# ZhangT-tech/MoCA-Video

Hardware: AMD Instinct MI355X
Metric: denoising UNet-steps/sec @16x320x512 fp16 (higher is better)
Workload: dtype f16

## Files before the change

### include/moca_hip.h

```cpp
#ifndef MOCA_HIP_H
#define MOCA_HIP_H

#include <stdint.h>

#ifdef __cplusplus
extern "C" {
#endif

#define MOCA_OK            0
#define MOCA_E_BADARG     -1
#define MOCA_E_LAUNCH     -2
#define MOCA_E_NODEVICE   -3
#define MOCA_E_GRAPH      -4

#define MOCA_A_LINEAR   0
#define MOCA_A_CONV3X3  1
#define MOCA_A_TCONV3   2

#define MOCA_EP_GEGLU   1
#define MOCA_EP_OUT_F32 2
#define MOCA_FORCE_SMALL_TILE 4
#define MOCA_EP_COLSUM 16
#define MOCA_EP_LN     32
#define MOCA_EP_GELU    8
// ... 227 lines not shown
int moca_base_ddim_step_f32(moca_fifo_state* state, float* x, const float* eps_c, const float* eps_u, const float* noise,
                            float* pred_x0, const float* coef, int32_t S, float cfg_scale, int32_t use_scale, int64_t n, void* stream);
int moca_mask_frame_sums_f32(const float* mask, float* sums, int32_t frames, int32_t HW, void* stream);

int moca_freq_mix_3d_f32(const float* x, const float* noise, const float* lpf, float* out,
                         int32_t C, int32_t T, int32_t H, int32_t W, float* ws, void* stream);
int64_t moca_freq_mix_ws_bytes(int32_t C, int32_t T, int32_t H, int32_t W);
int moca_freq_filter_f32(float* lpf, int32_t T, int32_t H, int32_t W, int32_t type, int32_t n,
                         double d_s, double d_t, void* stream);

int moca_graph_begin(void* stream);
int moca_graph_end(void* stream, void** graph_exec_out);
int moca_graph_launch(void* graph_exec, void* stream);
int moca_graph_destroy(void* graph_exec);
int moca_stream_create(void** stream_out);
int moca_stream_destroy(void* stream);
int moca_stream_sync(void* stream);
int moca_event_create(void** ev_out);
int moca_event_record(void* ev, void* stream);
int moca_event_elapsed_ms(void* ev_start, void* ev_stop, float* ms_out);
int moca_event_destroy(void* ev);

#define MOCA_TUNE_GEMM_W80   0
#define MOCA_TUNE_GEMM_G4    1
#define MOCA_TUNE_GEMM_SQ256 2
#define MOCA_TUNE_GEMM_WIDE  3
#define MOCA_TUNE_GN_SLAB    4
#define MOCA_TUNE_GEMM_G4P   5
#define MOCA_TUNE_GEMM_MF32  6
#define MOCA_TUNE_GEMM_SQP   7
#define MOCA_TUNE_SQP_WALK   8
#define MOCA_TUNE_SLAB_F16   9
#define MOCA_TUNE_GEMM_WS    10
#define MOCA_TUNE_COUNT      11
int moca_set_tuning(int32_t knob, int32_t value);
int moca_debug_clock_sampler(void* buf, int32_t blocks, int32_t nsamples, const int32_t* stop, void* stream);

int moca_device_info(char* name, int32_t len, int32_t* cu_count);
const char* moca_version(void);

#ifdef __cplusplus
}
#endif
#endif
```

### moca_video_amd/csrc/norm.hip

```cpp
#include "common.h"

namespace {

constexpr int GN_GROUPS = 32;

__host__ __device__ inline int gn_nchunk(int F, int HW) {
    int n = 2048 / (F > 0 ? F : 1);
    if (n < 1) n = 1;
    const int maxc = (HW + 7) / 8;
    if (n > maxc) n = maxc;
    if (n < 1) n = 1;
    return n;
}

__global__ void gn_partial_kernel(const half_t* __restrict__ x, float* __restrict__ partial,
                                  int HW, int C, int nchunk) {
    extern __shared__ __attribute__((aligned(16))) char smem_raw[];
    float* s_sum = reinterpret_cast<float*>(smem_raw);
    float* s_sq = s_sum + blockDim.y * C;
    const int f = blockIdx.x, chunk = blockIdx.y;
    const int cx = threadIdx.x, py = threadIdx.y, ppb = blockDim.y;
    const int pc = (HW + nchunk - 1) / nchunk;
    const int p_begin = chunk * pc, p_end = min(p_begin + pc, HW);
    float s[8], q[8];
#pragma unroll
    for (int j = 0; j < 8; ++j) { s[j] = 0.f; q[j] = 0.f; }
    const half_t* base = x + ((int64_t)f * HW) * C + cx * 8;
    int pp = p_begin + py;
    for (; pp + 3 * ppb < p_end; pp += 4 * ppb) {
        half8v v[4];
#pragma unroll
        for (int u = 0; u < 4; ++u) v[u] = *reinterpret_cast<const half8v*>(base + (int64_t)(pp + u * ppb) * C);
#pragma unroll
        for (int u = 0; u < 4; ++u)
#pragma unroll
            for (int j = 0; j < 8; ++j) { const float a = (float)v[u][j]; s[j] += a; q[j] += a * a; }
    }
    for (; pp < p_end; pp += ppb) {
        const half8v v = *reinterpret_cast<const half8v*>(base + (int64_t)pp * C);
#pragma unroll
        for (int j = 0; j < 8; ++j) { const float a = (float)v[j]; s[j] += a; q[j] += a * a; }
    }
#pragma unroll
    for (int j = 0; j < 8; ++j) { s_sum[py * C + cx * 8 + j] = s[j]; s_sq[py * C + cx * 8 + j] = q[j]; }
    __syncthreads();
    const int tid = py * blockDim.x + cx;
// ... 37 lines not shown
        float2 v[4];
#pragma unroll
        for (int u = 0; u < 4; ++u) {
            const int i = i0 + u * FIN_T;
            v[u] = i < n ? *reinterpret_cast<const float2*>(base + ((int64_t)i * GN_GROUPS + g) * 2) : float2{0.f, 0.f};
        }
#pragma unroll
        for (int u = 0; u < 4; ++u) { a += (double)v[u].x; b += (double)v[u].y; }
    }
    gn_finalize_store(a, b, meanrstd, (int64_t)sg * GN_GROUPS + g, inv_count, eps);
}

__global__ __launch_bounds__(FIN_T) void gn_finalize_colsum_kernel(const float* __restrict__ colsum, float* __restrict__ meanrstd,
                                                                   int tps, int C, int cpg, double inv_count, float eps) {
    const int sg = blockIdx.x, g = blockIdx.y, l = threadIdx.x;
    const int n = tps * cpg;
    double a = 0.0, b = 0.0;
    for (int i0 = l; i0 < n; i0 += 4 * FIN_T) {
        float2 v[4];
#pragma unroll
        for (int u = 0; u < 4; ++u) {
            const int i = i0 + u * FIN_T;
            const int t = i / cpg, c = g * cpg + (i - t * cpg);
            v[u] = i < n ? *reinterpret_cast<const float2*>(colsum + (((int64_t)sg * tps + t) * C + c) * 2) : float2{0.f, 0.f};
        }
#pragma unroll
        for (int u = 0; u < 4; ++u) { a += (double)v[u].x; b += (double)v[u].y; }
    }
    gn_finalize_store(a, b, meanrstd, (int64_t)sg * GN_GROUPS + g, inv_count, eps);
}

__global__ void gn_apply_kernel(const half_t* __restrict__ x, half_t* __restrict__ y,
                                const float* __restrict__ gamma, const float* __restrict__ beta,
                                const float* __restrict__ meanrstd, int HW, int C, int nchunk,
                                int frames_per_stat, int silu) {
    const int f = blockIdx.x, chunk = blockIdx.y;
    const int cx = threadIdx.x, py = threadIdx.y, ppb = blockDim.y;
    const int pc = (HW + nchunk - 1) / nchunk;
    const int p_begin = chunk * pc, p_end = min(p_begin + pc, HW);
    if (p_begin >= p_end) return;
    const int cpg = C / GN_GROUPS;
    const int sg = f / frames_per_stat;
    const int64_t off = ((int64_t)f * HW) * C + cx * 8;
    auto load4 = [&](half8v (&v)[4], int pp) {
#pragma unroll
        for (int u = 0; u < 4; ++u) v[u] = *reinterpret_cast<const half8v*>(x + off + (int64_t)min(pp + u * ppb, p_end - 1) * C);
    };
    int pp = p_begin + py;
    half8v cur[4], nxt[4];
    load4(cur, pp);
    float sc[8], sh[8];
#pragma unroll
    for (int j = 0; j < 8; ++j) {
        const int c = cx * 8 + j;
        const int g = c / cpg;
        const float mean = meanrstd[((int64_t)sg * GN_GROUPS + g) * 2];
        const float rstd = meanrstd[((int64_t)sg * GN_GROUPS + g) * 2 + 1];
        sc[j] = rstd * gamma[c];
        sh[j] = beta[c] - mean * sc[j];
    }
    auto norm8 = [&](const half8v& v) {
        half8v o;
#pragma unroll
        for (int j = 0; j < 8; ++j) {
            float a = (float)v[j] * sc[j] + sh[j];
            if (silu) a = moca_silu(a);
            o[j] = (half_t)a;
        }
        return o;
    };
    for (; pp < p_end; pp += 4 * ppb) {
        const bool more = pp + 4 * ppb < p_end;
        if (more) load4(nxt, pp + 4 * ppb);
#pragma unroll
        for (int u = 0; u < 4; ++u)
            if (pp + u * ppb < p_end) *reinterpret_cast<half8v*>(y + off + (int64_t)(pp + u * ppb) * C) = norm8(cur[u]);
        if (more) {
#pragma unroll
            for (int u = 0; u < 4; ++u) cur[u] = nxt[u];
        }
    }
}

template <bool STREAM>
__device__ __forceinline__ void gn_st8(half_t* ptr, const half8v v) {
    if constexpr (STREAM) __builtin_nontemporal_store(v, reinterpret_cast<half8v*>(ptr));
    else *reinterpret_cast<half8v*>(ptr) = v;
}
template <bool STREAM>
__global__ void gn_apply_gstat_kernel(const half_t* __restrict__ x, half_t* __restrict__ y,
                                      const float* __restrict__ gamma, const float* __restrict__ beta,
                                      const int64_t* __restrict__ gstat, int HW, int C, int nchunk,
                                      int frames_per_stat, double inv_count, float eps, int silu) {
    __shared__ float s_mr[2 * GN_GROUPS];
    const int f = blockIdx.x, chunk = blockIdx.y;
    const int cx = threadIdx.x, py = threadIdx.y, ppb = blockDim.y;
    const int tid = py * blockDim.x + cx;
    const int pc = (HW + nchunk - 1) / nchunk;
    const int p_begin = chunk * pc, p_end = min(p_begin + pc, HW);
    if (p_begin >= p_end) return;
    const int cpg = C / GN_GROUPS;
    const int sg = f / frames_per_stat;
    const int64_t off = ((int64_t)f * HW) * C + cx * 8;
    auto load4 = [&](half8v (&v)[4], int pp) {
#pragma unroll
        for (int u = 0; u < 4; ++u) v[u] = *reinterpret_cast<const half8v*>(x + off + (int64_t)min(pp + u * ppb, p_end - 1) * C);
    };
    int pp = p_begin + py;
    half8v cur[4], nxt[4];
    load4(cur, pp);
    const f32x4 gm0 = *reinterpret_cast<const f32x4*>(gamma + cx * 8), gm1 = *reinterpret_cast<const f32x4*>(gamma + cx * 8 + 4);
    const f32x4 bt0 = *reinterpret_cast<const f32x4*>(beta + cx * 8), bt1 = *reinterpret_cast<const f32x4*>(beta + cx * 8 + 4);
    if (tid < GN_GROUPS) {
        const double a = moca_gstat_get(gstat + ((int64_t)sg * GN_GROUPS + tid) * 2, 0), b = moca_gstat_get(gstat + ((int64_t)sg * GN_GROUPS + tid) * 2 + 1, 1);
        const double mean = a * inv_count;
        double var = b * inv_count - mean * mean;
        if (var < 0.0) var = 0.0;
        s_mr[2 * tid] = (float)mean;
        s_mr[2 * tid + 1] = (float)(1.0 / sqrt(var + (double)eps));
    }
    __syncthreads();
    float sc[8], sh[8];
#pragma unroll
    for (int j = 0; j < 8; ++j) {
        const int c = cx * 8 + j;
        const int g = c / cpg;
        sc[j] = s_mr[2 * g + 1] * (j < 4 ? gm0[j & 3] : gm1[j & 3]);
        sh[j] = (j < 4 ? bt0[j & 3] : bt1[j & 3]) - s_mr[2 * g] * sc[j];
    }
    auto norm8 = [&](const half8v& v) {
        half8v o;
#pragma unroll
        for (int j = 0; j < 8; ++j) {
            float a = (float)v[j] * sc[j] + sh[j];
            if (silu) a = moca_silu(a);
            o[j] = (half_t)a;
// ... 38 lines not shown
        for (int u = 0; u < 4; ++u) v[u] = *reinterpret_cast<const half8v*>(src + (int64_t)(pp + u * ppb) * ld);
#pragma unroll
        for (int u = 0; u < 4; ++u) {
            gn_st8<STREAM>(dst + (int64_t)(pp + u * ppb) * C, v[u]);
#pragma unroll
            for (int j = 0; j < 8; ++j) { const float t = (float)v[u][j]; s[j] += t; q[j] += t * t; }
        }
    }
    for (; pp < p_end; pp += ppb) {
        const half8v v = *reinterpret_cast<const half8v*>(src + (int64_t)pp * ld);
        gn_st8<STREAM>(dst + (int64_t)pp * C, v);
#pragma unroll
        for (int j = 0; j < 8; ++j) { const float t = (float)v[j]; s[j] += t; q[j] += t * t; }
    }
#pragma unroll
    for (int j = 0; j < 8; ++j) { s_sum[py * C + cx * 8 + j] = s[j]; s_sq[py * C + cx * 8 + j] = q[j]; }
    __syncthreads();
    const int tid = py * blockDim.x + cx;
    if (tid < 2 * GN_GROUPS) {
        const int g = tid >> 1, comp = tid & 1;
        const int cpg = C / GN_GROUPS;
        const float* base = comp ? s_sq : s_sum;
        float t = 0.f;
        for (int y = 0; y < ppb; ++y)
            for (int c = g * cpg; c < (g + 1) * cpg; ++c) t += base[y * C + c];
        moca_gstat_add(gstat + ((int64_t)(f / frames_per_stat) * GN_GROUPS + g) * 2 + comp, comp, t);
    }
}

template <bool STREAM>
__global__ void gn_apply_gstat_cat_kernel(const half_t* __restrict__ a, const half_t* __restrict__ b, half_t* __restrict__ y,
                                          const float* __restrict__ gamma, const float* __restrict__ beta,
                                          const int64_t* __restrict__ gstat_cat, const int64_t* __restrict__ gstat_b,
                                          int HW, int C1, int C2, int nchunk, int frames_per_stat, int sgb_mod, double inv_count, float eps, int silu) {
    __shared__ float s_mr[2 * GN_GROUPS];
    const int C = C1 + C2;
    const int f = blockIdx.x, chunk = blockIdx.y;
    const int cx = threadIdx.x, py = threadIdx.y, ppb = blockDim.y;
    const int tid = py * blockDim.x + cx;
    const int pc = (HW + nchunk - 1) / nchunk;
    const int p_begin = chunk * pc, p_end = min(p_begin + pc, HW);
    if (p_begin >= p_end) return;
    const int cpg = C / GN_GROUPS;
    const int sg = f / frames_per_stat;
    const bool from_a = cx * 8 < C1;
    const half_t* src = from_a ? a + ((int64_t)f * HW) * C1 + cx * 8 : b + ((int64_t)f * HW) * C2 + (cx * 8 - C1);
    const int ld = from_a ? C1 : C2;
    const int64_t off = ((int64_t)f * HW) * C + cx * 8;
    auto load4 = [&](half8v (&v)[4], int pp) {
#pragma unroll
        for (int u = 0; u < 4; ++u) v[u] = *reinterpret_cast<const half8v*>(src + (int64_t)min(pp + u * ppb, p_end - 1) * ld);
    };
    int pp = p_begin + py;
    half8v cur[4], nxt[4];
    load4(cur, pp);
    const f32x4 gm0 = *reinterpret_cast<const f32x4*>(gamma + cx * 8), gm1 = *reinterpret_cast<const f32x4*>(gamma + cx * 8 + 4);
    const f32x4 bt0 = *reinterpret_cast<const f32x4*>(beta + cx * 8), bt1 = *reinterpret_cast<const f32x4*>(beta + cx * 8 + 4);
    if (tid < GN_GROUPS) {
        const int64_t* ga = gstat_cat + ((int64_t)sg * GN_GROUPS + tid) * 2;
        double sa = moca_gstat_get(ga, 0), sq = moca_gstat_get(ga + 1, 1);
        if (gstat_b) {
            const int cpg2 = C2 / GN_GROUPS;
            const int lo = max(tid * cpg - C1, 0), hi = min((tid + 1) * cpg - C1, C2);
            for (int j = lo / cpg2; j * cpg2 < hi; ++j) {
                const int64_t* gb = gstat_b + ((int64_t)(sg % sgb_mod) * GN_GROUPS + j) * 2;
                sa += moca_gstat_get(gb, 0); sq += moca_gstat_get(gb + 1, 1);
            }
        }
        const double mean = sa * inv_count;
        double var = sq * inv_count - mean * mean;
        if (var < 0.0) var = 0.0;
        s_mr[2 * tid] = (float)mean;
        s_mr[2 * tid + 1] = (float)(1.0 / sqrt(var + (double)eps));
    }
    __syncthreads();
    float sc[8], sh[8];
#pragma unroll
    for (int j = 0; j < 8; ++j) {
        const int c = cx * 8 + j;
        const int g = c / cpg;
        sc[j] = s_mr[2 * g + 1] * (j < 4 ? gm0[j & 3] : gm1[j & 3]);
// ... 107 lines not shown
        if (var < 0.0) var = 0.0;
        const float rstd = (float)(1.0 / sqrt(var + (double)eps));
        const float sc = rstd * gm_t;
        s_sc[tid] = sc;
        s_sh[tid] = bt_t - (float)mean * sc;
    }
    __syncthreads();
    const int rps = (R + S - 1) / S;
    const int r0 = split * rps, r1 = min(R, r0 + rps);
    half_t* ys = y + base;
    {
        int row = r0 + tid / vpr, v = tid % vpr;
#pragma unroll 2
        for (; row < r1;) {
            const int64_t o = (int64_t)row * C + v * VEC;
            const vec_t d = *reinterpret_cast<const vec_t*>(xs + o);
            vec_t r;
#pragma unroll
            for (int j = 0; j < VEC; ++j) {
                float a = (float)d[j] * s_sc[v * VEC + j] + s_sh[v * VEC + j];
                if (silu) a = moca_silu(a);
                r[j] = (half_t)a;
            }
            *reinterpret_cast<vec_t*>(ys + o) = r;
            row += dr; v += dv;
            if (v >= vpr) { v -= vpr; ++row; }
        }
    }
}

template <int CPT>
__global__ __launch_bounds__(1024) void gn_slab_reg_kernel(const half_t* __restrict__ x, half_t* __restrict__ y,
                                                            const float* __restrict__ gamma, const float* __restrict__ beta,
                                                            int R, int C, int cpg, double inv_count, float eps, int silu) {
    __shared__ float s_red[2][16];
    __shared__ float s_sc[128], s_sh[128];
    const int tid = threadIdx.x, nthr = blockDim.x;
    const int slab = blockIdx.x, sg = slab / GN_GROUPS, g = slab % GN_GROUPS;
    const int vpr = cpg / 8, nchunks = R * vpr;
    const int64_t base = (int64_t)sg * R * C + g * cpg;
    const float gm_t = tid < cpg ? gamma[g * cpg + tid] : 0.f, bt_t = tid < cpg ? beta[g * cpg + tid] : 0.f;
    half8v v[CPT];
    int off[CPT];
    float s = 0.f, q = 0.f;
#pragma unroll
    for (int i = 0; i < CPT; ++i) {
        const int idx = tid + i * nthr;
        off[i] = -1;
        if (idx < nchunks) {
            const int row = idx / vpr, c = idx - row * vpr;
            off[i] = row * C + c * 8;
            v[i] = *reinterpret_cast<const half8v*>(x + base + off[i]);
        }
    }
#pragma unroll
    for (int i = 0; i < CPT; ++i)
        if (off[i] >= 0) {
#pragma unroll
            for (int j = 0; j < 8; ++j) { const float a = (float)v[i][j]; s += a; q += a * a; }
        }
    s = wave_sum(s); q = wave_sum(q);
    if ((tid & 63) == 0) { s_red[0][tid >> 6] = s; s_red[1][tid >> 6] = q; }
    __syncthreads();
    if (tid < cpg) {
        double a = 0.0, b = 0.0;
        for (int w = 0; w < (nthr >> 6); ++w) { a += (double)s_red[0][w]; b += (double)s_red[1][w]; }
        const double mean = a * inv_count;
        double var = b * inv_count - mean * mean;
        if (var < 0.0) var = 0.0;
        const float rstd = (float)(1.0 / sqrt(var + (double)eps));
        const float sc = rstd * gm_t;
        s_sc[tid] = sc;
        s_sh[tid] = bt_t - (float)mean * sc;
    }
    __syncthreads();
#pragma unroll
    for (int i = 0; i < CPT; ++i)
        if (off[i] >= 0) {
            const int c0 = (off[i] % C);
            half8v r;
#pragma unroll
            for (int j = 0; j < 8; ++j) {
                float a = (float)v[i][j] * s_sc[c0 + j] + s_sh[c0 + j];
                if (silu) a = moca_silu(a);
                r[j] = (half_t)a;
            }
            *reinterpret_cast<half8v*>(y + base + off[i]) = r;
        }
}

template <int MAXCH, int LN_ROWS>
__global__ __launch_bounds__(256) void layernorm_kernel(const half_t* __restrict__ x, half_t* __restrict__ y,
                                                        const float* __restrict__ gamma, const float* __restrict__ beta,
                                                        int M, int C, float eps) {
    const int lane = threadIdx.x & 63, wave = threadIdx.x >> 6;
    const int row0 = (blockIdx.x * 4 + wave) * LN_ROWS;
    if (row0 >= M) return;
    const int nch = C / 8;
    half8v v[LN_ROWS][MAXCH];
#pragma unroll
    for (int r = 0; r < LN_ROWS; ++r) {
        const int row = min(row0 + r, M - 1);
        const half_t* xr = x + (int64_t)row * C;
#pragma unroll
        for (int i = 0; i < MAXCH; ++i) {
            const int ch = lane + 64 * i;
            if (ch < nch) v[r][i] = *reinterpret_cast<const half8v*>(xr + ch * 8);
        }
    }
    float mean[LN_ROWS], rstd[LN_ROWS];
#pragma unroll
// ... 27 lines not shown
        if (ch < nch) {
            const f32x4 g0 = *reinterpret_cast<const f32x4*>(gamma + ch * 8), g1 = *reinterpret_cast<const f32x4*>(gamma + ch * 8 + 4);
            const f32x4 b0 = *reinterpret_cast<const f32x4*>(beta + ch * 8), b1 = *reinterpret_cast<const f32x4*>(beta + ch * 8 + 4);
#pragma unroll
            for (int r = 0; r < LN_ROWS; ++r) {
                if (row0 + r < M) {
                    half8v o;
#pragma unroll
                    for (int j = 0; j < 4; ++j) {
                        o[j] = (half_t)(((float)v[r][i][j] - mean[r]) * rstd[r] * g0[j] + b0[j]);
                        o[4 + j] = (half_t)(((float)v[r][i][4 + j] - mean[r]) * rstd[r] * g1[j] + b1[j]);
                    }
                    *reinterpret_cast<half8v*>(y + (int64_t)(row0 + r) * C + ch * 8) = o;
                }
            }
        }
    }
}

}

extern "C" int64_t moca_groupnorm_ws_bytes(int32_t F, int32_t HW, int32_t C) {
    (void)C;
    const int nchunk = gn_nchunk(F, HW);
    return ((int64_t)F * nchunk * GN_GROUPS * 2 + (int64_t)F * GN_GROUPS * 2) * 4;
}

extern "C" int moca_groupnorm_nhwc_f16(const void* x, void* y, const float* gamma, const float* beta,
                                       int32_t F, int32_t HW, int32_t C, int32_t frames_per_stat,
                                       float eps, int32_t silu, float* ws, void* stream) {
    if (!x || !y || !gamma || !beta || !ws) return MOCA_E_BADARG;
    if (F <= 0 || HW <= 0 || C <= 0 || C % (8 * 1) || C % GN_GROUPS || frames_per_stat <= 0 || F % frames_per_stat) return MOCA_E_BADARG;
    const int nch8 = C / 8;
    if (nch8 > 1024) return MOCA_E_BADARG;
    int ppb = 256 / nch8;
    if (ppb < 1) ppb = 1;
    const int nchunk = gn_nchunk(F, HW);
    float* partial = ws;
    float* meanrstd = ws + (int64_t)F * nchunk * GN_GROUPS * 2;
    hipStream_t st = moca_stream(stream);
    const double inv_count = 1.0 / ((double)frames_per_stat * HW * (C / GN_GROUPS));
    {
        const int slab_mode = moca_tuning_get(MOCA_TUNE_GN_SLAB);
        const int cpg = C / GN_GROUPS;
        const int64_t bytes = (int64_t)F * HW * C * 2;
        const int64_t R64 = (int64_t)frames_per_stat * HW;
        if (slab_mode && cpg % 2 == 0 && cpg <= 128 && R64 < (1 << 24) &&
            (slab_mode == 2 || bytes <= (8 << 20) || (frames_per_stat == 1 && HW <= 160 && bytes <= (28 << 20)))) {
            const int R = (int)R64;
            const int n_slabs = (F / frames_per_stat) * GN_GROUPS;
            {
                const int nchunks = R * (cpg / 8);
                if (cpg % 8 == 0 && nchunks <= 4096 && nchunks >= 256) {
                    const int cpt = (nchunks + 1023) / 1024;
                    const int thr = ((nchunks + cpt - 1) / cpt + 63) / 64 * 64;
                    const half_t* xi = reinterpret_cast<const half_t*>(x);
                    half_t* yo = reinterpret_cast<half_t*>(y);
#define MOCA_SLABREG(CPT) hipLaunchKernelGGL(gn_slab_reg_kernel<CPT>, dim3(n_slabs), dim3(thr), 0, st, xi, yo, gamma, beta, R, C, cpg, inv_count, eps, silu)
                    if (cpt == 1) MOCA_SLABREG(1); else if (cpt == 2) MOCA_SLABREG(2); else if (cpt == 3) MOCA_SLABREG(3); else MOCA_SLABREG(4);
#undef MOCA_SLABREG
                    MOCA_CHECK_LAUNCH();
                    return MOCA_OK;
                }
            }
            int S = 1024 / n_slabs;
            if (S > 16) S = 16;
            if (S > R) S = R;
            if (S < 1) S = 1;
            const int xcd_map = (n_slabs % 8 == 0) ? 1 : 0;
            const dim3 g1(n_slabs * S), b1(256);
            const half_t* xi = reinterpret_cast<const half_t*>(x);
            half_t* yo = reinterpret_cast<half_t*>(y);
            if (cpg % 8 == 0)
                hipLaunchKernelGGL(gn_slab_kernel<8>, g1, b1, 0, st, xi, yo, gamma, beta, R, C, cpg, S, xcd_map, inv_count, eps, silu);
            else if (cpg % 4 == 0)
                hipLaunchKernelGGL(gn_slab_kernel<4>, g1, b1, 0, st, xi, yo, gamma, beta, R, C, cpg, S, xcd_map, inv_count, eps, silu);
            else
                hipLaunchKernelGGL(gn_slab_kernel<2>, g1, b1, 0, st, xi, yo, gamma, beta, R, C, cpg, S, xcd_map, inv_count, eps, silu);
            MOCA_CHECK_LAUNCH();
            return MOCA_OK;
        }
    }
    const dim3 grid(F, nchunk), block(nch8, ppb);
    const size_t lds = (size_t)ppb * C * 2 * sizeof(float);
    hipLaunchKernelGGL(gn_partial_kernel, grid, block, lds, st, reinterpret_cast<const half_t*>(x), partial, HW, C, nchunk);
    MOCA_CHECK_LAUNCH();
    hipLaunchKernelGGL(gn_finalize_kernel, dim3(F / frames_per_stat, GN_GROUPS), dim3(FIN_T), 0, st, partial, meanrstd,
                       frames_per_stat, nchunk, inv_count, eps);
    MOCA_CHECK_LAUNCH();
    hipLaunchKernelGGL(gn_apply_kernel, grid, block, 0, st, reinterpret_cast<const half_t*>(x), reinterpret_cast<half_t*>(y),
                       gamma, beta, meanrstd, HW, C, nchunk, frames_per_stat, silu);
    MOCA_CHECK_LAUNCH();
    return MOCA_OK;
}

extern "C" int moca_groupnorm_colsum_f16(const void* x, void* y, const float* gamma, const float* beta, const float* colsum,
                                         int32_t tile_rows, int32_t F, int32_t HW, int32_t C, int32_t frames_per_stat,
                                         float eps, int32_t silu, float* ws, void* stream) {
    if (!x || !y || !gamma || !beta || !ws || !colsum) return MOCA_E_BADARG;
    if (F <= 0 || HW <= 0 || C <= 0 || C % 8 || C % GN_GROUPS || frames_per_stat <= 0 || F % frames_per_stat) return MOCA_E_BADARG;
    if (tile_rows <= 0 || ((int64_t)frames_per_stat * HW) % tile_rows) return MOCA_E_BADARG;
    const int nch8 = C / 8;
    if (nch8 > 1024) return MOCA_E_BADARG;
    int ppb = 256 / nch8;
    if (ppb < 1) ppb = 1;
    const int nchunk = gn_nchunk(F, HW);
    float* meanrstd = ws + (int64_t)F * nchunk * GN_GROUPS * 2;
    hipStream_t st = moca_stream(stream);
    const double inv_count = 1.0 / ((double)frames_per_stat * HW * (C / GN_GROUPS));
    const int tps = (int)(((int64_t)frames_per_stat * HW) / tile_rows);
    hipLaunchKernelGGL(gn_finalize_colsum_kernel, dim3(F / frames_per_stat, GN_GROUPS), dim3(FIN_T), 0, st, colsum, meanrstd,
                       tps, C, C / GN_GROUPS, inv_count, eps);
    MOCA_CHECK_LAUNCH();
    const dim3 grid(F, nchunk), block(nch8, ppb);
    hipLaunchKernelGGL(gn_apply_kernel, grid, block, 0, st, reinterpret_cast<const half_t*>(x), reinterpret_cast<half_t*>(y),
                       gamma, beta, meanrstd, HW, C, nchunk, frames_per_stat, silu);
    MOCA_CHECK_LAUNCH();
    return MOCA_OK;
}

extern "C" int moca_groupnorm_gstat_f16(const void* x, void* y, const float* gamma, const float* beta, const int64_t* gstat,
                                        int32_t F, int32_t HW, int32_t C, int32_t frames_per_stat,
                                        float eps, int32_t silu, void* stream) {
    if (!x || !y || !gamma || !beta || !gstat) return MOCA_E_BADARG;
    if ((reinterpret_cast<uintptr_t>(gamma) | reinterpret_cast<uintptr_t>(beta)) & 15) return MOCA_E_BADARG;
    if (F <= 0 || HW <= 0 || C <= 0 || C % 8 || C % GN_GROUPS || frames_per_stat <= 0 || F % frames_per_stat) return MOCA_E_BADARG;
    const int nch8 = C / 8;
    if (nch8 > 1024) return MOCA_E_BADARG;
    int ppb = 256 / nch8;
    if (ppb < 1) ppb = 1;
    if (nch8 * ppb < GN_GROUPS) return MOCA_E_BADARG;
    const int nchunk = gn_nchunk(F, HW);
    const double inv_count = 1.0 / ((double)frames_per_stat * HW * (C / GN_GROUPS));
    const dim3 grid(F, nchunk), block(nch8, ppb);
    const bool streams = (int64_t)F * HW * C * 2 >= (128ll << 20);
    hipLaunchKernelGGL(streams ? gn_apply_gstat_kernel<true> : gn_apply_gstat_kernel<false>, grid, block, 0, moca_stream(stream),
                       reinterpret_cast<const half_t*>(x), reinterpret_cast<half_t*>(y), gamma, beta, gstat, HW, C, nchunk, frames_per_stat,
                       inv_count, eps, silu);
    MOCA_CHECK_LAUNCH();
    return MOCA_OK;
}

__global__ __launch_bounds__(256) void gn_fold_weights_kernel(const half_t* __restrict__ w, const float* __restrict__ bias,
                                                              const float* __restrict__ gamma, const float* __restrict__ beta,
                                                              const int64_t* __restrict__ gstat, half_t* __restrict__ wg, float* __restrict__ bg,
                                                              int N, int K, int ldw, double inv_count, float eps) {
    extern __shared__ float s_st[];
    const int sg = blockIdx.x, tid = threadIdx.x;
    const int cpg = K / GN_GROUPS;
    __shared__ float s_mr[2 * GN_GROUPS];
    if (tid < GN_GROUPS) {
        const double a = moca_gstat_get(gstat + ((int64_t)sg * GN_GROUPS + tid) * 2, 0), b = moca_gstat_get(gstat + ((int64_t)sg * GN_GROUPS + tid) * 2 + 1, 1);
        const double mean = a * inv_count;
        double var = b * inv_count - mean * mean;
        if (var < 0.0) var = 0.0;
        s_mr[2 * tid] = (float)mean;
        s_mr[2 * tid + 1] = (float)(1.0 / sqrt(var + (double)eps));
    }
    __syncthreads();
    for (int k = tid; k < K; k += 256) {
        const int g = k / cpg;
        s_st[k] = s_mr[2 * g + 1] * gamma[k];
        s_st[K + k] = beta[k];
    }
    __syncthreads();
    const int cpr = ldw / 8;
    float* s_dot = s_st + 2 * K;
    const int rows_pb = 16;
    const int n0 = blockIdx.y * rows_pb;
    for (int idx = tid; idx < rows_pb * cpr; idx += 256) {
// ... 42 lines not shown
    const int C = C1 + C2;
    if (C % GN_GROUPS || frames_per_stat <= 0 || F % frames_per_stat) return MOCA_E_BADARG;
    const int nch8 = C / 8;
    if (nch8 > 1024) return MOCA_E_BADARG;
    int ppb = 256 / nch8;
    if (ppb < 1) ppb = 1;
    if (nch8 * ppb < 2 * GN_GROUPS) return MOCA_E_BADARG;
    const int nchunk = gn_nchunk(F, HW);
    const size_t lds = (size_t)ppb * C * 2 * sizeof(float);
    if (lds > 64 * 1024) return MOCA_E_BADARG;
    const bool streams = (int64_t)F * HW * C * 2 >= (128ll << 20);
    hipLaunchKernelGGL(streams ? concat_gstat_kernel<true> : concat_gstat_kernel<false>, dim3(F, nchunk), dim3(nch8, ppb), lds, moca_stream(stream),
                       reinterpret_cast<const half_t*>(a), reinterpret_cast<const half_t*>(b), reinterpret_cast<half_t*>(out), gstat, HW, C1, C2,
                       nchunk, frames_per_stat);
    MOCA_CHECK_LAUNCH();
    return MOCA_OK;
}

extern "C" int moca_groupnorm_gstat_cat_f16(const void* a, const void* b, void* y, const float* gamma, const float* beta,
                                            const int64_t* gstat_cat, const int64_t* gstat_b, int32_t Fb, int32_t F, int32_t HW, int32_t C1,
                                            int32_t C2, int32_t frames_per_stat, float eps, int32_t silu, void* stream) {
    if (!a || !b || !y || !gamma || !beta || !gstat_cat) return MOCA_E_BADARG;
    if ((reinterpret_cast<uintptr_t>(gamma) | reinterpret_cast<uintptr_t>(beta)) & 15) return MOCA_E_BADARG;
    if (Fb <= 0) Fb = F;
    if (Fb > F || F % Fb || Fb % frames_per_stat) return MOCA_E_BADARG;
    if (F <= 0 || HW <= 0 || C1 <= 0 || C2 <= 0 || C1 % 8 || C2 % 8 || frames_per_stat <= 0 || F % frames_per_stat) return MOCA_E_BADARG;
    const int C = C1 + C2;
    if (C % GN_GROUPS) return MOCA_E_BADARG;
    if (gstat_b) {
        const int cpg = C / GN_GROUPS, cpg2 = C2 / GN_GROUPS;
        if (C2 % GN_GROUPS || cpg % cpg2 || (C1 % cpg) % cpg2) return MOCA_E_BADARG;
    }
    const int nch8 = C / 8;
    if (nch8 > 1024) return MOCA_E_BADARG;
    int ppb = 256 / nch8;
    if (ppb < 1) ppb = 1;
    if (nch8 * ppb < GN_GROUPS) return MOCA_E_BADARG;
    const int nchunk = gn_nchunk(F, HW);
    const double inv_count = 1.0 / ((double)frames_per_stat * HW * (C / GN_GROUPS));
    const dim3 grid(F, nchunk), block(nch8, ppb);
    const bool streams = (int64_t)F * HW * C * 2 >= (128ll << 20);
    hipLaunchKernelGGL(streams ? gn_apply_gstat_cat_kernel<true> : gn_apply_gstat_cat_kernel<false>, grid, block, 0, moca_stream(stream),
                       reinterpret_cast<const half_t*>(a), reinterpret_cast<const half_t*>(b), reinterpret_cast<half_t*>(y), gamma, beta,
                       gstat_cat, gstat_b, HW, C1, C2, nchunk, frames_per_stat, Fb / frames_per_stat, inv_count, eps, silu);
    MOCA_CHECK_LAUNCH();
    return MOCA_OK;
}

extern "C" int moca_gstat_accum_f16(const void* x, int32_t F, int32_t HW, int32_t C, int32_t frames_per_stat, int32_t cpg, int32_t coff,
                                    int64_t* gstat, void* stream) {
    if (!x || !gstat || F <= 0 || HW <= 0 || C <= 0 || C % 8 || frames_per_stat <= 0 || F % frames_per_stat) return MOCA_E_BADARG;
    if (cpg <= 0 || coff < 0 || (coff + C - 1) / cpg >= GN_GROUPS) return MOCA_E_BADARG;
    const int nch8 = C / 8;
    if (nch8 > 1024) return MOCA_E_BADARG;
    int ppb = 256 / nch8;
    if (ppb < 1) ppb = 1;
    if (nch8 * ppb < 2 * ((coff + C - 1) / cpg - coff / cpg + 1)) return MOCA_E_BADARG;
    const int nchunk = gn_nchunk(F, HW);
    const size_t lds = (size_t)ppb * C * 2 * sizeof(float);
    if (lds > 64 * 1024) return MOCA_E_BADARG;
    hipLaunchKernelGGL(gstat_accum_kernel, dim3(F, nchunk), dim3(nch8, ppb), lds, moca_stream(stream),
                       reinterpret_cast<const half_t*>(x), gstat, HW, C, nchunk, frames_per_stat, cpg, coff);
    MOCA_CHECK_LAUNCH();
    return MOCA_OK;
}

extern "C" int moca_layernorm_f16(const void* x, void* y, const float* gamma, const float* beta,
                                  int32_t M, int32_t C, float eps, void* stream) {
    if (!x || !y || !gamma || !beta || M <= 0 || C <= 0 || C % 8) return MOCA_E_BADARG;
    const int nch = C / 8;
    hipStream_t st = moca_stream(stream);
    const half_t* xi = reinterpret_cast<const half_t*>(x);
    half_t* yo = reinterpret_cast<half_t*>(y);
    const dim3 block(256);
#define MOCA_LN(MAXCH, ROWS) hipLaunchKernelGGL((layernorm_kernel<MAXCH, ROWS>), dim3((M + 4 * ROWS - 1) / (4 * ROWS)), block, 0, st, xi, yo, gamma, beta, M, C, eps)
    if (M >= 16384) {
        if (nch <= 64) MOCA_LN(1, 4);
// ... 16 lines not shown
```

### moca_video_amd/csrc/runtime.hip

```cpp
#include "common.h"
#include <string.h>
#include <stdio.h>
#include <stdlib.h>

extern "C" int moca_graph_begin(void* stream) {
    if (hipStreamBeginCapture(moca_stream(stream), hipStreamCaptureModeThreadLocal) != hipSuccess) return MOCA_E_GRAPH;
    return MOCA_OK;
}

extern "C" int moca_graph_end(void* stream, void** graph_exec_out) {
    if (!graph_exec_out) return MOCA_E_BADARG;
    hipGraph_t g = nullptr;
    if (hipStreamEndCapture(moca_stream(stream), &g) != hipSuccess || !g) return MOCA_E_GRAPH;
    hipGraphExec_t ge = nullptr;
    hipError_t e = hipGraphInstantiate(&ge, g, nullptr, nullptr, 0);
    (void)hipGraphDestroy(g);
    if (e != hipSuccess || !ge) return MOCA_E_GRAPH;
    *graph_exec_out = reinterpret_cast<void*>(ge);
    return MOCA_OK;
}

extern "C" int moca_graph_launch(void* graph_exec, void* stream) {
    if (!graph_exec) return MOCA_E_BADARG;
    if (hipGraphLaunch(reinterpret_cast<hipGraphExec_t>(graph_exec), moca_stream(stream)) != hipSuccess) return MOCA_E_GRAPH;
// ... 65 lines not shown
    const int64_t n16 = bytes / 16;
    int blocks = (int)((n16 + 255) / 256);
    if (blocks < 1) blocks = 1;
    if (blocks > 1024) blocks = 1024;
    hipLaunchKernelGGL(zero_kernel, dim3(blocks), dim3(256), 0, moca_stream(stream), reinterpret_cast<uint4*>(ptr), n16,
                       reinterpret_cast<unsigned char*>(ptr) + n16 * 16, (int)(bytes - n16 * 16));
    MOCA_CHECK_LAUNCH();
    return MOCA_OK;
}

__global__ __launch_bounds__(64) void clock_sampler_kernel(unsigned long long* __restrict__ buf, int nsamples, const volatile int* stop) {
#if defined(__HIP_DEVICE_COMPILE__)
    if (threadIdx.x) return;
    unsigned long long* b = buf + (size_t)blockIdx.x * nsamples * 2;
    for (int i = 0; i < nsamples; ++i) {
        unsigned long long t, r;
        asm volatile("s_memtime %0\n\ts_memrealtime %1\n\ts_waitcnt lgkmcnt(0)" : "=s"(t), "=s"(r)::"memory");
        b[2 * i] = t;
        b[2 * i + 1] = r;
        if (stop && *stop) break;
        __builtin_amdgcn_s_sleep(127);
        __builtin_amdgcn_s_sleep(127);
    }
#endif
}
extern "C" int moca_debug_clock_sampler(void* buf, int32_t blocks, int32_t nsamples, const int32_t* stop, void* stream) {
    if (!buf || blocks < 1 || blocks > 64 || nsamples < 1 || nsamples > (1 << 20)) return MOCA_E_BADARG;
    hipLaunchKernelGGL(clock_sampler_kernel, dim3(blocks), dim3(64), 0, moca_stream(stream), reinterpret_cast<unsigned long long*>(buf), nsamples,
                       reinterpret_cast<const volatile int*>(stop));
    MOCA_CHECK_LAUNCH();
    return MOCA_OK;
}

static int g_tuning[MOCA_TUNE_COUNT] = {1, 1, 1, 1, 1, 1, 0, 1, 0, 0, 1};
int moca_tuning_get(int knob) { return (knob >= 0 && knob < MOCA_TUNE_COUNT) ? g_tuning[knob] : 0; }
extern "C" int moca_set_tuning(int32_t knob, int32_t value) {
    if (knob < 0 || knob >= MOCA_TUNE_COUNT || value < 0 || value > 2) return MOCA_E_BADARG;
    const int old = g_tuning[knob];
    g_tuning[knob] = value;
    return old;
}
```

### moca_video_amd/lib.py

```python
from __future__ import annotations

import ctypes as C
import os

import torch

_HERE = os.path.dirname(os.path.abspath(__file__))
LIB_PATH = os.environ.get("MOCA_HIP_LIB") or os.path.join(_HERE, "libmoca_hip.so")

MOCA_A_LINEAR, MOCA_A_CONV3X3, MOCA_A_TCONV3 = 0, 1, 2
MOCA_EP_GEGLU, MOCA_EP_OUT_F32, MOCA_FORCE_SMALL_TILE, MOCA_EP_GELU, MOCA_EP_COLSUM, MOCA_EP_LN = 1, 2, 4, 8, 16, 32
MOCA_EP_ROWSUM, MOCA_EP_LNFOLD, MOCA_EP_GSTAT, MOCA_EP_TATTN, MOCA_EP_SLABS = 64, 128, 256, 512, 1024
MOCA_TUNE_GEMM_W80, MOCA_TUNE_GEMM_G4, MOCA_TUNE_GEMM_SQ256, MOCA_TUNE_GEMM_WIDE, MOCA_TUNE_GN_SLAB, MOCA_TUNE_GEMM_G4P, MOCA_TUNE_GEMM_MF32, MOCA_TUNE_GEMM_SQP, MOCA_TUNE_SQP_WALK = 0, 1, 2, 3, 4, 5, 6, 7, 8
MOCA_TUNE_SLAB_F16 = 9
MOCA_TUNE_GEMM_WS = 10
(MOCA_ROUTE_SMALL64, MOCA_ROUTE_SMALL128, MOCA_ROUTE_GLDS128, MOCA_ROUTE_GLDS160, MOCA_ROUTE_G4, MOCA_ROUTE_W80, MOCA_ROUTE_W80W,
 MOCA_ROUTE_SQ256, MOCA_ROUTE_G4P, MOCA_ROUTE_SQP, MOCA_ROUTE_TATTN, MOCA_ROUTE_WS) = range(1, 13)

_ERR = {0: "ok", -1: "bad argument (shape/alignment contract)", -2: "HIP launch/runtime error",
        -3: "no gfx950 device", -4: "graph capture/replay failed"}


class MocaHipError(RuntimeError):
    pass


class GemmParams(C.Structure):
    _fields_ = [
        ("a", C.c_void_p), ("w", C.c_void_p), ("out", C.c_void_p), ("bias", C.c_void_p),
        ("rowadd", C.c_void_p), ("residual", C.c_void_p), ("splitk_ws", C.c_void_p),
        ("M", C.c_int32), ("N", C.c_int32), ("K", C.c_int32),
        ("lda", C.c_int32), ("ldw", C.c_int32), ("ldo", C.c_int32), ("ldr", C.c_int32), ("ld_rowadd", C.c_int32),
        ("rowadd_div", C.c_int32), ("a_mode", C.c_int32), ("C", C.c_int32),
        ("inH", C.c_int32), ("inW", C.c_int32), ("outH", C.c_int32), ("outW", C.c_int32),
        ("stride", C.c_int32), ("up", C.c_int32), ("T", C.c_int32), ("HW", C.c_int32),
        ("flags", C.c_int32), ("splits", C.c_int32), ("nopad_lo", C.c_int32), ("prefetch_kib", C.c_int32),
        ("tattn_causal", C.c_int32),
        ("colsum", C.c_void_p), ("ln_gamma", C.c_void_p), ("ln_beta", C.c_void_p), ("ln_out", C.c_void_p),
        ("ld_ln", C.c_int32), ("ln_eps", C.c_float),
        ("rowsum", C.c_void_p), ("lnf_part", C.c_void_p), ("lnf_wsum", C.c_void_p),
        ("lnf_nparts", C.c_int32), ("reserved2_", C.c_int32),
        ("gstat", C.c_void_p), ("gstat_rows", C.c_int32), ("tattn_scale", C.c_float),
        ("prefetch", C.c_void_p), ("up_phase", C.c_int32), ("reserved4_", C.c_int32),
        ("a2", C.c_void_p), ("lda2", C.c_int32), ("k1", C.c_int32), ("gstat_cpg", C.c_int32), ("gstat_coff", C.c_int32),
        ("wgroup_rows", C.c_int32), ("wgroup_stride", C.c_int32),
    ]


# ... 154 lines not shown
```

Before: 60.25.

## Regrid GroupNorm apply over stat groups and split slab-register kernel across blocks

```diff
diff --git a/include/moca_hip.h b/include/moca_hip.h
--- a/include/moca_hip.h
+++ b/include/moca_hip.h
@@ -283,7 +283,8 @@
 #define MOCA_TUNE_SQP_WALK   8
 #define MOCA_TUNE_SLAB_F16   9
 #define MOCA_TUNE_GEMM_WS    10
-#define MOCA_TUNE_COUNT      11
+#define MOCA_TUNE_GN_SLAB_SPLIT 11
+#define MOCA_TUNE_COUNT      12
 int moca_set_tuning(int32_t knob, int32_t value);
 int moca_debug_clock_sampler(void* buf, int32_t blocks, int32_t nsamples, const int32_t* stop, void* stream);
 
diff --git a/moca_video_amd/csrc/norm.hip b/moca_video_amd/csrc/norm.hip
--- a/moca_video_amd/csrc/norm.hip
+++ b/moca_video_amd/csrc/norm.hip
@@ -12,6 +12,33 @@
     if (n < 1) n = 1;
     return n;
 }
+
+struct GnApplyGeom { int ppb, R, rpb, bpsg, gps; dim3 grid; };
+inline GnApplyGeom gn_apply_geom(int nch8, int F, int HW, int fps) {
+    GnApplyGeom g;
+    int a = nch8, b = 64;
+    while (b) { const int t = a % b; a = b; b = t; }
+    g.ppb = 64 / a;
+    g.ppb *= (256 + nch8 * g.ppb - 1) / (nch8 * g.ppb);
+    if (nch8 * g.ppb > 512) g.ppb = 256 / nch8 > 0 ? 256 / nch8 : 1;
+    g.R = fps * HW; g.gps = 1;
+    g.rpb = 4 * g.ppb;
+    g.bpsg = (g.R + g.rpb - 1) / g.rpb;
+    if ((int64_t)(F / fps) * g.bpsg <= 2048) {
+        g.grid = dim3((F / fps) * g.bpsg);
+        return g;
+    }
+    const int nchunk = gn_nchunk(F, HW);
+    g.ppb = 256 / nch8 > 0 ? 256 / nch8 : 1;
+    g.R = HW; g.gps = fps;
+    g.rpb = (HW + nchunk - 1) / nchunk;
+    g.bpsg = nchunk;
+    g.grid = dim3(F, nchunk);
+    return g;
+}
+#define GN_APPLY_BLOCK() \
+    const int grp = gridDim.y > 1 ? blockIdx.x : blockIdx.x / bpsg, blk = gridDim.y > 1 ? blockIdx.y : blockIdx.x - grp * bpsg; \
+    const int sg = grp / gps
 
 __global__ void gn_partial_kernel(const half_t* __restrict__ x, float* __restrict__ partial,
                                   int HW, int C, int nchunk) {
@@ -115,16 +142,13 @@
 
 __global__ void gn_apply_kernel(const half_t* __restrict__ x, half_t* __restrict__ y,
                                 const float* __restrict__ gamma, const float* __restrict__ beta,
-                                const float* __restrict__ meanrstd, int HW, int C, int nchunk,
-                                int frames_per_stat, int silu) {
-    const int f = blockIdx.x, chunk = blockIdx.y;
+                                const float* __restrict__ meanrstd, int R, int C, int rpb, int bpsg, int gps, int silu) {
+    GN_APPLY_BLOCK();
     const int cx = threadIdx.x, py = threadIdx.y, ppb = blockDim.y;
-    const int pc = (HW + nchunk - 1) / nchunk;
-    const int p_begin = chunk * pc, p_end = min(p_begin + pc, HW);
+    const int p_begin = blk * rpb, p_end = min(p_begin + rpb, R);
     if (p_begin >= p_end) return;
     const int cpg = C / GN_GROUPS;
-    const int sg = f / frames_per_stat;
-    const int64_t off = ((int64_t)f * HW) * C + cx * 8;
+    const int64_t off = ((int64_t)grp * R) * C + cx * 8;
     auto load4 = [&](half8v (&v)[4], int pp) {
 #pragma unroll
         for (int u = 0; u < 4; ++u) v[u] = *reinterpret_cast<const half8v*>(x + off + (int64_t)min(pp + u * ppb, p_end - 1) * C);
@@ -173,18 +197,16 @@
 template <bool STREAM>
 __global__ void gn_apply_gstat_kernel(const half_t* __restrict__ x, half_t* __restrict__ y,
                                       const float* __restrict__ gamma, const float* __restrict__ beta,
-                                      const int64_t* __restrict__ gstat, int HW, int C, int nchunk,
-                                      int frames_per_stat, double inv_count, float eps, int silu) {
+                                      const int64_t* __restrict__ gstat, int R, int C, int rpb, int bpsg, int gps,
+                                      double inv_count, float eps, int silu) {
     __shared__ float s_mr[2 * GN_GROUPS];
-    const int f = blockIdx.x, chunk = blockIdx.y;
+    GN_APPLY_BLOCK();
     const int cx = threadIdx.x, py = threadIdx.y, ppb = blockDim.y;
     const int tid = py * blockDim.x + cx;
-    const int pc = (HW + nchunk - 1) / nchunk;
-    const int p_begin = chunk * pc, p_end = min(p_begin + pc, HW);
+    const int p_begin = blk * rpb, p_end = min(p_begin + rpb, R);
     if (p_begin >= p_end) return;
     const int cpg = C / GN_GROUPS;
-    const int sg = f / frames_per_stat;
-    const int64_t off = ((int64_t)f * HW) * C + cx * 8;
+    const int64_t off = ((int64_t)grp * R) * C + cx * 8;
     auto load4 = [&](half8v (&v)[4], int pp) {
 #pragma unroll
         for (int u = 0; u < 4; ++u) v[u] = *reinterpret_cast<const half8v*>(x + off + (int64_t)min(pp + u * ppb, p_end - 1) * C);
@@ -289,21 +311,19 @@
 __global__ void gn_apply_gstat_cat_kernel(const half_t* __restrict__ a, const half_t* __restrict__ b, half_t* __restrict__ y,
                                           const float* __restrict__ gamma, const float* __restrict__ beta,
                                           const int64_t* __restrict__ gstat_cat, const int64_t* __restrict__ gstat_b,
-                                          int HW, int C1, int C2, int nchunk, int frames_per_stat, int sgb_mod, double inv_count, float eps, int silu) {
+                                          int R, int C1, int C2, int rpb, int bpsg, int gps, int sgb_mod, double inv_count, float eps, int silu) {
     __shared__ float s_mr[2 * GN_GROUPS];
     const int C = C1 + C2;
-    const int f = blockIdx.x, chunk = blockIdx.y;
+    GN_APPLY_BLOCK();
     const int cx = threadIdx.x, py = threadIdx.y, ppb = blockDim.y;
     const int tid = py * blockDim.x + cx;
-    const int pc = (HW + nchunk - 1) / nchunk;
-    const int p_begin = chunk * pc, p_end = min(p_begin + pc, HW);
+    const int p_begin = blk * rpb, p_end = min(p_begin + rpb, R);
     if (p_begin >= p_end) return;
     const int cpg = C / GN_GROUPS;
-    const int sg = f / frames_per_stat;
     const bool from_a = cx * 8 < C1;
-    const half_t* src = from_a ? a + ((int64_t)f * HW) * C1 + cx * 8 : b + ((int64_t)f * HW) * C2 + (cx * 8 - C1);
+    const half_t* src = from_a ? a + ((int64_t)grp * R) * C1 + cx * 8 : b + ((int64_t)grp * R) * C2 + (cx * 8 - C1);
     const int ld = from_a ? C1 : C2;
-    const int64_t off = ((int64_t)f * HW) * C + cx * 8;
+    const int64_t off = ((int64_t)grp * R) * C + cx * 8;
     auto load4 = [&](half8v (&v)[4], int pp) {
 #pragma unroll
         for (int u = 0; u < 4; ++u) v[u] = *reinterpret_cast<const half8v*>(src + (int64_t)min(pp + u * ppb, p_end - 1) * ld);
@@ -477,12 +497,16 @@
 template <int CPT>
 __global__ __launch_bounds__(1024) void gn_slab_reg_kernel(const half_t* __restrict__ x, half_t* __restrict__ y,
                                                             const float* __restrict__ gamma, const float* __restrict__ beta,
-                                                            int R, int C, int cpg, double inv_count, float eps, int silu) {
+                                                            int R, int C, int cpg, int S, int xcd_map, double inv_count, float eps, int silu) {
     __shared__ float s_red[2][16];
     __shared__ float s_sc[128], s_sh[128];
-    const int tid = threadIdx.x, nthr = blockDim.x;
-    const int slab = blockIdx.x, sg = slab / GN_GROUPS, g = slab % GN_GROUPS;
+    const int tid = threadIdx.x, nthr = blockDim.x, L = blockIdx.x;
+    int slab, split;
+    if (xcd_map) { const int w = L >> 3; slab = (L & 7) + 8 * (w / S); split = w % S; }
+    else { slab = L / S; split = L % S; }
+    const int sg = slab / GN_GROUPS, g = slab % GN_GROUPS;
     const int vpr = cpg / 8, nchunks = R * vpr;
+    const int st_lo = (int)((int64_t)split * nchunks / S), st_hi = (int)((int64_t)(split + 1) * nchunks / S);
     const int64_t base = (int64_t)sg * R * C + g * cpg;
     const float gm_t = tid < cpg ? gamma[g * cpg + tid] : 0.f, bt_t = tid < cpg ? beta[g * cpg + tid] : 0.f;
     half8v v[CPT];
@@ -521,7 +545,7 @@
     __syncthreads();
 #pragma unroll
     for (int i = 0; i < CPT; ++i)
-        if (off[i] >= 0) {
+        if (off[i] >= 0 && tid + i * nthr >= st_lo && tid + i * nthr < st_hi) {
             const int c0 = (off[i] % C);
             half8v r;
 #pragma unroll
@@ -615,7 +639,7 @@
     if (!x || !y || !gamma || !beta || !ws) return MOCA_E_BADARG;
     if (F <= 0 || HW <= 0 || C <= 0 || C % (8 * 1) || C % GN_GROUPS || frames_per_stat <= 0 || F % frames_per_stat) return MOCA_E_BADARG;
     const int nch8 = C / 8;
-    if (nch8 > 1024) return MOCA_E_BADARG;
+    if (nch8 > 1024 || (int64_t)frames_per_stat * HW >= (1ll << 31)) return MOCA_E_BADARG;
     int ppb = 256 / nch8;
     if (ppb < 1) ppb = 1;
     const int nchunk = gn_nchunk(F, HW);
@@ -635,11 +659,16 @@
             {
                 const int nchunks = R * (cpg / 8);
                 if (cpg % 8 == 0 && nchunks <= 4096 && nchunks >= 256) {
-                    const int cpt = (nchunks + 1023) / 1024;
-                    const int thr = ((nchunks + cpt - 1) / cpt + 63) / 64 * 64;
+                    const int cpt = nchunks >= 1024 ? 4 : (nchunks + 255) / 256;
+                    int thr = ((nchunks + cpt - 1) / cpt + 63) / 64 * 64;
+                    if (thr < (cpg + 63) / 64 * 64) thr = (cpg + 63) / 64 * 64;
+                    const int split_mode = moca_tuning_get(MOCA_TUNE_GN_SLAB_SPLIT);
+                    int S = split_mode ? split_mode : (n_slabs >= 256 ? 1 : (256 / n_slabs > 4 ? 4 : 256 / n_slabs));
+                    if (S > nchunks) S = nchunks;
+                    const int xcd_map = (n_slabs % 8 == 0) ? 1 : 0;
                     const half_t* xi = reinterpret_cast<const half_t*>(x);
                     half_t* yo = reinterpret_cast<half_t*>(y);
-#define MOCA_SLABREG(CPT) hipLaunchKernelGGL(gn_slab_reg_kernel<CPT>, dim3(n_slabs), dim3(thr), 0, st, xi, yo, gamma, beta, R, C, cpg, inv_count, eps, silu)
+#define MOCA_SLABREG(CPT) hipLaunchKernelGGL(gn_slab_reg_kernel<CPT>, dim3(n_slabs * S), dim3(thr), 0, st, xi, yo, gamma, beta, R, C, cpg, S, xcd_map, inv_count, eps, silu)
                     if (cpt == 1) MOCA_SLABREG(1); else if (cpt == 2) MOCA_SLABREG(2); else if (cpt == 3) MOCA_SLABREG(3); else MOCA_SLABREG(4);
 #undef MOCA_SLABREG
                     MOCA_CHECK_LAUNCH();
@@ -671,8 +700,9 @@
     hipLaunchKernelGGL(gn_finalize_kernel, dim3(F / frames_per_stat, GN_GROUPS), dim3(FIN_T), 0, st, partial, meanrstd,
                        frames_per_stat, nchunk, inv_count, eps);
     MOCA_CHECK_LAUNCH();
-    hipLaunchKernelGGL(gn_apply_kernel, grid, block, 0, st, reinterpret_cast<const half_t*>(x), reinterpret_cast<half_t*>(y),
-                       gamma, beta, meanrstd, HW, C, nchunk, frames_per_stat, silu);
+    const GnApplyGeom ag = gn_apply_geom(nch8, F, HW, frames_per_stat);
+    hipLaunchKernelGGL(gn_apply_kernel, ag.grid, dim3(nch8, ag.ppb), 0, st, reinterpret_cast<const half_t*>(x),
+                       reinterpret_cast<half_t*>(y), gamma, beta, meanrstd, ag.R, C, ag.rpb, ag.bpsg, ag.gps, silu);
     MOCA_CHECK_LAUNCH();
     return MOCA_OK;
 }
@@ -684,9 +714,7 @@
     if (F <= 0 || HW <= 0 || C <= 0 || C % 8 || C % GN_GROUPS || frames_per_stat <= 0 || F % frames_per_stat) return MOCA_E_BADARG;
     if (tile_rows <= 0 || ((int64_t)frames_per_stat * HW) % tile_rows) return MOCA_E_BADARG;
     const int nch8 = C / 8;
-    if (nch8 > 1024) return MOCA_E_BADARG;
-    int ppb = 256 / nch8;
-    if (ppb < 1) ppb = 1;
+    if (nch8 > 1024 || (int64_t)frames_per_stat * HW >= (1ll << 31)) return MOCA_E_BADARG;
     const int nchunk = gn_nchunk(F, HW);
     float* meanrstd = ws + (int64_t)F * nchunk * GN_GROUPS * 2;
     hipStream_t st = moca_stream(stream);
@@ -695,9 +723,9 @@
     hipLaunchKernelGGL(gn_finalize_colsum_kernel, dim3(F / frames_per_stat, GN_GROUPS), dim3(FIN_T), 0, st, colsum, meanrstd,
                        tps, C, C / GN_GROUPS, inv_count, eps);
     MOCA_CHECK_LAUNCH();
-    const dim3 grid(F, nchunk), block(nch8, ppb);
-    hipLaunchKernelGGL(gn_apply_kernel, grid, block, 0, st, reinterpret_cast<const half_t*>(x), reinterpret_cast<half_t*>(y),
-                       gamma, beta, meanrstd, HW, C, nchunk, frames_per_stat, silu);
+    const GnApplyGeom ag = gn_apply_geom(nch8, F, HW, frames_per_stat);
+    hipLaunchKernelGGL(gn_apply_kernel, ag.grid, dim3(nch8, ag.ppb), 0, st, reinterpret_cast<const half_t*>(x),
+                       reinterpret_cast<half_t*>(y), gamma, beta, meanrstd, ag.R, C, ag.rpb, ag.bpsg, ag.gps, silu);
     MOCA_CHECK_LAUNCH();
     return MOCA_OK;
 }
@@ -709,16 +737,14 @@
     if ((reinterpret_cast<uintptr_t>(gamma) | reinterpret_cast<uintptr_t>(beta)) & 15) return MOCA_E_BADARG;
     if (F <= 0 || HW <= 0 || C <= 0 || C % 8 || C % GN_GROUPS || frames_per_stat <= 0 || F % frames_per_stat) return MOCA_E_BADARG;
     const int nch8 = C / 8;
-    if (nch8 > 1024) return MOCA_E_BADARG;
-    int ppb = 256 / nch8;
-    if (ppb < 1) ppb = 1;
-    if (nch8 * ppb < GN_GROUPS) return MOCA_E_BADARG;
-    const int nchunk = gn_nchunk(F, HW);
+    if (nch8 > 1024 || (int64_t)frames_per_stat * HW >= (1ll << 31)) return MOCA_E_BADARG;
+    const GnApplyGeom ag = gn_apply_geom(nch8, F, HW, frames_per_stat);
+    if (nch8 * ag.ppb < GN_GROUPS) return MOCA_E_BADARG;
     const double inv_count = 1.0 / ((double)frames_per_stat * HW * (C / GN_GROUPS));
-    const dim3 grid(F, nchunk), block(nch8, ppb);
+    const dim3 block(nch8, ag.ppb);
     const bool streams = (int64_t)F * HW * C * 2 >= (128ll << 20);
-    hipLaunchKernelGGL(streams ? gn_apply_gstat_kernel<true> : gn_apply_gstat_kernel<false>, grid, block, 0, moca_stream(stream),
-                       reinterpret_cast<const half_t*>(x), reinterpret_cast<half_t*>(y), gamma, beta, gstat, HW, C, nchunk, frames_per_stat,
+    hipLaunchKernelGGL(streams ? gn_apply_gstat_kernel<true> : gn_apply_gstat_kernel<false>, ag.grid, block, 0, moca_stream(stream),
+                       reinterpret_cast<const half_t*>(x), reinterpret_cast<half_t*>(y), gamma, beta, gstat, ag.R, C, ag.rpb, ag.bpsg, ag.gps,
                        inv_count, eps, silu);
     MOCA_CHECK_LAUNCH();
     return MOCA_OK;
@@ -827,17 +853,15 @@
         if (C2 % GN_GROUPS || cpg % cpg2 || (C1 % cpg) % cpg2) return MOCA_E_BADARG;
     }
     const int nch8 = C / 8;
-    if (nch8 > 1024) return MOCA_E_BADARG;
-    int ppb = 256 / nch8;
-    if (ppb < 1) ppb = 1;
-    if (nch8 * ppb < GN_GROUPS) return MOCA_E_BADARG;
-    const int nchunk = gn_nchunk(F, HW);
+    if (nch8 > 1024 || (int64_t)frames_per_stat * HW >= (1ll << 31)) return MOCA_E_BADARG;
+    const GnApplyGeom ag = gn_apply_geom(nch8, F, HW, frames_per_stat);
+    if (nch8 * ag.ppb < GN_GROUPS) return MOCA_E_BADARG;
     const double inv_count = 1.0 / ((double)frames_per_stat * HW * (C / GN_GROUPS));
-    const dim3 grid(F, nchunk), block(nch8, ppb);
+    const dim3 block(nch8, ag.ppb);
     const bool streams = (int64_t)F * HW * C * 2 >= (128ll << 20);
-    hipLaunchKernelGGL(streams ? gn_apply_gstat_cat_kernel<true> : gn_apply_gstat_cat_kernel<false>, grid, block, 0, moca_stream(stream),
+    hipLaunchKernelGGL(streams ? gn_apply_gstat_cat_kernel<true> : gn_apply_gstat_cat_kernel<false>, ag.grid, block, 0, moca_stream(stream),
                        reinterpret_cast<const half_t*>(a), reinterpret_cast<const half_t*>(b), reinterpret_cast<half_t*>(y), gamma, beta,
-                       gstat_cat, gstat_b, HW, C1, C2, nchunk, frames_per_stat, Fb / frames_per_stat, inv_count, eps, silu);
+                       gstat_cat, gstat_b, ag.R, C1, C2, ag.rpb, ag.bpsg, ag.gps, Fb / frames_per_stat, inv_count, eps, silu);
     MOCA_CHECK_LAUNCH();
     return MOCA_OK;
 }
diff --git a/moca_video_amd/csrc/runtime.hip b/moca_video_amd/csrc/runtime.hip
--- a/moca_video_amd/csrc/runtime.hip
+++ b/moca_video_amd/csrc/runtime.hip
@@ -121,7 +121,7 @@
     return MOCA_OK;
 }
 
-static int g_tuning[MOCA_TUNE_COUNT] = {1, 1, 1, 1, 1, 1, 0, 1, 0, 0, 1};
+static int g_tuning[MOCA_TUNE_COUNT] = {1, 1, 1, 1, 1, 1, 0, 1, 0, 0, 1, 0};
 int moca_tuning_get(int knob) { return (knob >= 0 && knob < MOCA_TUNE_COUNT) ? g_tuning[knob] : 0; }
 extern "C" int moca_set_tuning(int32_t knob, int32_t value) {
     if (knob < 0 || knob >= MOCA_TUNE_COUNT || value < 0 || value > 2) return MOCA_E_BADARG;
diff --git a/moca_video_amd/lib.py b/moca_video_amd/lib.py
--- a/moca_video_amd/lib.py
+++ b/moca_video_amd/lib.py
@@ -14,6 +14,7 @@
 MOCA_TUNE_GEMM_W80, MOCA_TUNE_GEMM_G4, MOCA_TUNE_GEMM_SQ256, MOCA_TUNE_GEMM_WIDE, MOCA_TUNE_GN_SLAB, MOCA_TUNE_GEMM_G4P, MOCA_TUNE_GEMM_MF32, MOCA_TUNE_GEMM_SQP, MOCA_TUNE_SQP_WALK = 0, 1, 2, 3, 4, 5, 6, 7, 8
 MOCA_TUNE_SLAB_F16 = 9
 MOCA_TUNE_GEMM_WS = 10
+MOCA_TUNE_GN_SLAB_SPLIT = 11
 (MOCA_ROUTE_SMALL64, MOCA_ROUTE_SMALL128, MOCA_ROUTE_GLDS128, MOCA_ROUTE_GLDS160, MOCA_ROUTE_G4, MOCA_ROUTE_W80, MOCA_ROUTE_W80W,
  MOCA_ROUTE_SQ256, MOCA_ROUTE_G4P, MOCA_ROUTE_SQP, MOCA_ROUTE_TATTN, MOCA_ROUTE_WS) = range(1, 13)
 
```

Result: no change. 60.42, median of 6 (+0.3%).
